# fengpeng-yue/speech-to-speech-translation

Hardware: AMD Instinct MI355X
Metric: mel-frames/sec (fwd+bwd+opt) on Fisher-shaped fbank80->mel80 (higher is better)
Workload: dtype bf16; 1 GPU; s2st_transformer base 12enc/6dec d512 nfps4 + aux ASR/ST(1x64) + CTC, recipe dropouts, max-tokens=20000 Fisher-shaped batches, update-freq 1; parallelism=dp1

## Files before the change

include/s2st_hip.h:

```cpp
#ifndef S2ST_HIP_H
#define S2ST_HIP_H
#include <stdint.h>
#ifdef __cplusplus
extern "C" {
#endif

#define S2ST_OK 0
#define S2ST_ERR_LAUNCH (-1)
#define S2ST_ERR_SHAPE (-2)
#define S2ST_ERR_WORKSPACE (-3)
#define S2ST_ERR_ARG (-4)
#define S2ST_ERR_COMM (-5)

typedef struct { int64_t ld; int64_t bs; int32_t per; int32_t _pad; } s2st_split;

typedef struct {
  const void* p;
  int32_t kmajor;
  int32_t dtype;
  s2st_split sp;
  int64_t zo, zi;
} s2st_gemm_operand;

#define S2ST_F32 0
// ... 90 lines not shown

int s2st_add_pe_f32(const float* x, float* y, const int32_t* pos, const float* table, int32_t rows, int32_t C, float scale, const float* alpha_ptr, float drop_p, uint64_t seed, void* stream);

int s2st_pe_alpha_bwd_f32(const float* dy, const int32_t* pos, const float* table, int32_t rows, int32_t C, float drop_p, uint64_t seed, float* dalpha, void* stream);

int s2st_embed_fwd_f32(const int64_t* tokens, const float* table, float* y, int32_t rows, int32_t C, float scale, void* stream);

int s2st_embed_bwd_f32(const int64_t* tokens, const float* dy, float* dtable, int32_t rows, int32_t C, float scale, int64_t pad, void* stream);
int s2st_embed_bwd_ordered_f32(const int64_t* tokens, const float* dy, float* dtable, int32_t rows, int32_t C, int32_t V, float scale, int64_t pad, void* stream);

int s2st_dropout_f32(const float* x, float* y, int64_t n, float a, float p, uint64_t seed, int32_t accumulate, void* stream);

int s2st_relu_drop_bwd_f32(const float* dy, const float* y, float* dz, int64_t n, float p, void* stream);

int s2st_conv_w_permute_f32(const float* w, float* wf, float* wd, int32_t O, int32_t I, int32_t Kw, void* stream);

int s2st_conv_w_unpermute_acc_f32(const float* dwf, float* dw, int32_t O, int32_t I, int32_t Kw, void* stream);

#define S2ST_BN_TMP_FLOATS(C) (130 * (long)(C))
int s2st_bn_stats_f32(const float* x, int32_t rows, int32_t C, float* mean, float* var, float* run_mean, float* run_var, float momentum, float* tmp, void* stream);

int s2st_bn_apply_f32(const float* x, const float* mean, const float* var, const float* gamma, const float* beta, float* y, s2st_split ysp, const float* resid, int32_t rows, int32_t C, float eps, int32_t tanh_, float drop_p, uint64_t seed, void* stream);

int s2st_bn_bwd_f32(const float* dy, s2st_split dysp, const float* x, const float* mean, const float* var, const float* gamma, const float* beta, float* dx, s2st_split dxsp, float* dgamma, float* dbeta, float* tmp, int32_t rows, int32_t C, float eps, int32_t tanh_, float drop_p, uint64_t seed, void* stream);

int s2st_bn_apply_img_f32(const float* x, const float* mean, const float* var, const float* gamma, const float* beta, float* y, uint16_t* img, int32_t B, int32_t T, int32_t pad, int32_t C, float eps, int32_t tanh_, float drop_p, uint64_t seed, void* stream);

int s2st_bn_stats_apply_f32(const float* x, int32_t rows, int32_t C, float* mean, float* var, float* run_mean, float* run_var, float momentum, float* tmp, const float* gamma, const float* beta, float* y, s2st_split ysp, const float* resid, float eps, int32_t tanh_, float drop_p, uint64_t seed, void* stream);
int s2st_bn_stats_apply_img_f32(const float* x, int32_t B, int32_t T, int32_t pad, int32_t C, float* mean, float* var, float* run_mean, float* run_var, float momentum, float* tmp, const float* gamma, const float* beta, float* y, uint16_t* img, float eps, int32_t tanh_, float drop_p, uint64_t seed, void* stream);

int s2st_bn_bwd_twin_f32(const float* dy, s2st_split dysp, const float* x, const float* mean, const float* var, const float* gamma, const float* beta, float* dx, s2st_split dxsp, float* dgamma, float* dbeta, float* tmp, int32_t rows, int32_t C, float eps, int32_t tanh_, float drop_p, uint64_t seed, uint16_t* dxh, int64_t ldh, void* stream);

// ... 317 lines not shown
```

speech-to-speech-translation_amd/csrc/c_api.cpp:

```cpp
#include <hip/hip_ext.h>
#include "s2st_ops.h"

extern "C" {

int s2st_version(void) { return 100; }

int s2st_experimental_build(void) {
#ifdef S2ST_EXPERIMENTAL
  return 1;
#else
  return 0;
#endif
}

int s2st_device_count(void) {
  int n = 0;
  if (hipGetDeviceCount(&n) != hipSuccess) return 0;
  return n;
}

int s2st_exchange_proxy_f32(const float* bucket, float* scratch, int64_t n, int64_t move_bytes, int32_t wgs, float gbps, void* stream) {
  return s2st_exchange_proxy(bucket, scratch, (long)n, (long)move_bytes, wgs, gbps, (hipStream_t)stream);
}
int s2st_grad_pack_bf16_f32(const float* g, uint16_t* out, int64_t n, void* stream) {
// ... 74 lines not shown
  return s2st_embed_bwd((const long*)tokens, dy, dtable, rows, C, scale, (long)pad, (hipStream_t)stream, V);
}

int s2st_dropout_f32(const float* x, float* y, int64_t n, float a, float p, uint64_t seed, int32_t accumulate, void* stream) {
  return s2st_dropout(x, y, n, a, p, seed, accumulate, (hipStream_t)stream);
}

int s2st_relu_drop_bwd_f32(const float* dy, const float* y, float* dz, int64_t n, float p, void* stream) {
  return s2st_relu_drop_bwd(dy, y, dz, n, p, (hipStream_t)stream);
}

int s2st_conv_w_permute_f32(const float* w, float* wf, float* wd, int32_t O, int32_t I, int32_t Kw, void* stream) {
  return s2st_conv_w_permute(w, wf, wd, O, I, Kw, (hipStream_t)stream);
}

int s2st_conv_w_unpermute_acc_f32(const float* dwf, float* dw, int32_t O, int32_t I, int32_t Kw, void* stream) {
  return s2st_conv_w_unpermute_acc(dwf, dw, O, I, Kw, (hipStream_t)stream);
}

int s2st_bn_stats_f32(const float* x, int32_t rows, int32_t C, float* mean, float* var, float* run_mean, float* run_var, float momentum, float* tmp, void* stream) {
  return s2st_bn_stats(x, rows, C, mean, var, run_mean, run_var, momentum, tmp, (hipStream_t)stream);
}

int s2st_bn_apply_f32(const float* x, const float* mean, const float* var, const float* gamma, const float* beta, float* y, s2st_split ysp, const float* resid, int32_t rows, int32_t C, float eps, int32_t tanh_, float drop_p, uint64_t seed, void* stream) {
  return s2st_bn_apply(x, mean, var, gamma, beta, y, ysp, resid, rows, C, eps, tanh_, drop_p, seed, (hipStream_t)stream);
}

int s2st_bn_bwd_f32(const float* dy, s2st_split dysp, const float* x, const float* mean, const float* var, const float* gamma, const float* beta, float* dx, s2st_split dxsp, float* dgamma, float* dbeta, float* tmp, int32_t rows, int32_t C, float eps, int32_t tanh_, float drop_p, uint64_t seed, void* stream) {
  return s2st_bn_bwd(dy, dysp, x, mean, var, gamma, beta, dx, dxsp, dgamma, dbeta, tmp, rows, C, eps, tanh_, drop_p, seed, (hipStream_t)stream);
}

int s2st_bn_apply_img_f32(const float* x, const float* mean, const float* var, const float* gamma, const float* beta, float* y, uint16_t* img, int32_t B, int32_t T, int32_t pad, int32_t C, float eps, int32_t tanh_, float drop_p, uint64_t seed, void* stream) {
// ... 259 lines not shown
```

speech-to-speech-translation_amd/csrc/elementwise.hip:

```cpp
#include <cstdlib>

#include "s2st_ops.h"
#include "s2st_prof.h"

namespace {

constexpr int EW_BLOCK = 256;

inline unsigned ew_grid(long n, int per_thread = 1) {
  long b = (n + (long)EW_BLOCK * per_thread - 1) / ((long)EW_BLOCK * per_thread);
  return (unsigned)(b < 1 ? 1 : b);
}

__global__ __launch_bounds__(256) void copy_rows_kernel(const float* __restrict__ x, Split xsp,
                                                        float* __restrict__ y, Split ysp, int rows,
                                                        int C4) {
  long i = (long)blockIdx.x * EW_BLOCK + threadIdx.x;
  long n = (long)rows * C4;
  if (i >= n) return;
  int r = (int)(i / C4), c = (int)(i - (long)r * C4);
  reinterpret_cast<float4*>(y + split_off(ysp, r))[c] =
      reinterpret_cast<const float4*>(x + split_off(xsp, r))[c];
}

// ... 408 lines not shown
    else atomicAdd(dbias + cc, v);
  }
}

__global__ __launch_bounds__(256) void axpy_kernel(const float* __restrict__ x,
                                                   float* __restrict__ y, long n, float a) {
  long i = (long)blockIdx.x * EW_BLOCK + threadIdx.x;
  if (i < n) y[i] += a * x[i];
}

__global__ __launch_bounds__(256) void scale_kernel(float* __restrict__ x, long n, float a) {
  long i = (long)blockIdx.x * EW_BLOCK + threadIdx.x;
  if (i < n) x[i] *= a;
}

__global__ __launch_bounds__(256) void conv_w_permute_kernel(const float* __restrict__ w,
                                                             float* __restrict__ wf,
                                                             float* __restrict__ wd, int O, int I,
                                                             int Kw, uint16_t* __restrict__ wfh,
                                                             uint16_t* __restrict__ wdh) {
  long i = (long)blockIdx.x * EW_BLOCK + threadIdx.x;
  long n = (long)O * I * Kw;
  if (i >= n) return;
  int j = (int)(i % Kw);
  int c = (int)((i / Kw) % I);
  int o = (int)(i / ((long)Kw * I));
  float v = w[i];
  const uint16_t vh = (uint16_t)(pack_bf16x4(v, 0.f, 0.f, 0.f).x & 0xffffu);
  if (wf) wf[((long)o * Kw + j) * I + c] = v;
  if (wd) wd[((long)c * Kw + (Kw - 1 - j)) * O + o] = v;
  if (wfh) wfh[((long)o * Kw + j) * I + c] = vh;
  if (wdh) wdh[((long)c * Kw + (Kw - 1 - j)) * O + o] = vh;
}

__global__ __launch_bounds__(256) void conv_w_permute_tiled_kernel(const float* __restrict__ w, float* __restrict__ wf,
                                                                   float* __restrict__ wd, int O, int I, int Kw,
                                                                   uint16_t* __restrict__ wfh, uint16_t* __restrict__ wdh) {
  __shared__ float tile[32][33];
  const int j = blockIdx.z, o0 = blockIdx.y * 32, c0 = blockIdx.x * 32;
  const int tx = threadIdx.x & 31, ty = threadIdx.x >> 5;
#pragma unroll
  for (int r = ty; r < 32; r += 8) {
    const int o = o0 + r, c = c0 + tx;
    float v = 0.f;
    if (o < O && c < I) {
      v = w[((long)o * I + c) * Kw + j];
      const long i = ((long)o * Kw + j) * I + c;
      if (wf) wf[i] = v;
      if (wfh) wfh[i] = (uint16_t)(pack_bf16x4(v, 0.f, 0.f, 0.f).x & 0xffffu);
    }
    tile[r][tx] = v;
  }
  __syncthreads();
  if (!wd && !wdh) return;
#pragma unroll
  for (int r = ty; r < 32; r += 8) {
    const int c = c0 + r, o = o0 + tx;
    if (o < O && c < I) {
      const float v = tile[tx][r];
      const long i = ((long)c * Kw + (Kw - 1 - j)) * O + o;
      if (wd) wd[i] = v;
      if (wdh) wdh[i] = (uint16_t)(pack_bf16x4(v, 0.f, 0.f, 0.f).x & 0xffffu);
    }
  }
}

__global__ __launch_bounds__(256) void conv_w_unpermute_acc_kernel(const float* __restrict__ dwf,
                                                                   float* __restrict__ dw, int O,
                                                                   int I, int Kw, int slabs) {
  long i = (long)blockIdx.x * EW_BLOCK + threadIdx.x;
  long n = (long)O * I * Kw;
  if (i >= n) return;
  int j = (int)(i % Kw);
  int c = (int)((i / Kw) % I);
  int o = (int)(i / ((long)Kw * I));
// ... 636 lines not shown
}

int s2st_axpy(const float* x, float* y, long n, float a, hipStream_t st) {
  if (n <= 0) return 0;
  S2ST_LAUNCH(axpy_kernel, dim3(ew_grid(n)), dim3(EW_BLOCK), 0, st, x, y, n, a);
  return LAUNCH_OK();
}

int s2st_scale(float* x, long n, float a, hipStream_t st) {
  if (n <= 0) return 0;
  S2ST_LAUNCH(scale_kernel, dim3(ew_grid(n)), dim3(EW_BLOCK), 0, st, x, n, a);
  return LAUNCH_OK();
}

int s2st_conv_w_permute(const float* w, float* wf, float* wd, int O, int I, int Kw, hipStream_t st, uint16_t* wfh,
                        uint16_t* wdh) {
  long n = (long)O * I * Kw;
  if (n <= 0) return 0;
  if (O >= 32 && I >= 32 && Kw <= 64) {
    S2ST_LAUNCH(conv_w_permute_tiled_kernel, dim3((I + 31) / 32, (O + 31) / 32, Kw), dim3(256), 0, st, w, wf, wd, O, I, Kw,
                wfh, wdh);
    return LAUNCH_OK();
  }
  S2ST_LAUNCH(conv_w_permute_kernel, dim3(ew_grid(n)), dim3(EW_BLOCK), 0, st, w, wf, wd, O, I, Kw, wfh, wdh);
  return LAUNCH_OK();
}

int s2st_conv_w_unpermute_acc(const float* dwf, float* dw, int O, int I, int Kw, hipStream_t st, int slabs) {
  long n = (long)O * I * Kw;
  if (n <= 0) return 0;
  S2ST_LAUNCH(conv_w_unpermute_acc_kernel, dim3(ew_grid(n)), dim3(EW_BLOCK), 0, st, dwf, dw, O, I, Kw, slabs < 1 ? 1 : slabs);
  return LAUNCH_OK();
}

int s2st_bn_stats(const float* x, int rows, int C, float* mean, float* var, float* run_mean,
                  float* run_var, float momentum, float* tmp, hipStream_t st) {
  if (rows <= 0 || C <= 0) return 0;
  int slabs = 0;
  int rc = colreduce2(ShiftSqF{x, C}, rows, C, nullptr, nullptr, tmp + 2 * (long)C, st, nullptr, nullptr, &slabs);
// ... 93 lines not shown
```

speech-to-speech-translation_amd/csrc/engine.cpp:

```cpp
#include <cmath>
#include <cstdio>
#include <cstdlib>
#include <cstring>
#include <functional>
#include <string>
#include <vector>

#include "s2st_ops.h"
#include <hip/hip_ext.h>

namespace {

struct PInfo {
  std::string name;
  long off, numel;
  int ndim;
  int shape[4];
  int is_buffer;
};

struct Ten {
  float* d = nullptr;
  float* g = nullptr;
  bf16raw* h = nullptr;
// ... 170 lines not shown
  float* dec_selfV(int l) const { return dec_selfK(l) + (long)dec_st.B * dec_st.maxT * c.dec_dim; }
  float* dec_crossKV(int l) const {
    return dec_st.base + (long)c.dec_layers * 2 * dec_st.B * dec_st.maxT * c.dec_dim + (long)l * dec_st.B * dec_st.E * 2 * c.dec_dim;
  }
  bool use_ln_skinny = true;
  bool use_skinny = true;
  bool use_ln_fuse = true;
  bool use_only_h = true;
  bool use_attn_gfuse = true;
  int attn_gfuse_mode = 1;
  bool ordered_sums = true;
  bool use_act_fuse = true;
  bool use_flash = true;
  bool attn_keep_f32 = s2st_env_on("S2ST_ATTN_KEEP_F32");
  bool convnet_fuse = s2st_env_int("S2ST_CONVNET_FUSE", 1) != 0;
  int ffn_act = 1;
  bool is_hubert = false;
  s2st_hubert_config hc{};
  struct HubP {
    long conv_w[8]; long gn_g, gn_b; LNP ln; LinP proj; long pos_w, pos_b; std::vector<EncLayerP> L; LNP enc_ln;
  } hp;
  float* ws_for(hipStream_t s) const { return (side_ && s == side_) ? skws_side : ((chain1_ && s == chain1_) ? skws_c1 : skws); }
  float* skws = nullptr;
  long skws_n = 0;
  bool ph_fresh = false;
  bf16raw* PHT = nullptr;
  bool pht_valid = false;
  struct WT { long off; int N, K; };
  std::vector<WT> wt_list;
  void reg_wt(long off, int N, int K) { if (N % 8 == 0 && K % 8 == 0) wt_list.push_back(WT{off, N, K}); }
// ... 650 lines not shown
```

speech-to-speech-translation_amd/csrc/engine_convnets.h:

```cpp
  ConvW make_conv_scratch(const ConvP& p, bool need_wd, bool tr) {
    ConvW s;
    const bool fm = fast();
    long n = (long)p.O * p.I * p.Kw;
    s.wf = fm ? nullptr : alloc(n);
    s.wd = (need_wd && !fm) ? alloc(n) : nullptr;
    s.dwf = alloc(n, tr);
    bf16raw* wfh = fm ? alloc_h((n + 7) / 8 * 8) : nullptr;
    bf16raw* wdh = fm && need_wd ? alloc_h((n + 7) / 8 * 8) : nullptr;
    if (live() && adam_pending && st_ != side_) adam_wait_upto(p.w + n);
    if (live()) chk(s2st_conv_w_permute(P + p.w, s.wf, s.wd, p.O, p.I, p.Kw, st_, wfh, wdh));
    s.wfh = wfh;
    s.wdh = wdh;
    return s;
  }

  bool bn_bwd_fusable(const Ten* z, int C) const { return fast() && convnet_fuse && C % 4 == 0 && z->hld() % 4 == 0; }
  bf16raw* bn_bwd_image(Ten* z, int B, int T) {
    if (!z->img_want || z->img_stride != 1 || z->img_B != B || z->img_Tout != T || z->img_Th != T + 2 * z->img_pad) return nullptr;
    z->gimg = alloc_h((long)B * z->img_Th * z->cols);
    return z->gimg;
  }

  Ten* postnet(Ten* feat, int B, int D, bool tr, std::vector<ConvW>& csp, float* post_out) {
    const bool fm = fast();
    Ten* cur = feat;
// ... 166 lines not shown
```

speech-to-speech-translation_amd/csrc/engine_ops.h:

```cpp
  Ten* linear(Ten* x, long w, long b, int N, int K, int act = 0, float drop_p = 0.f,
              Ten* resid = nullptr, float* ext_out = nullptr, bool only_h = false, const float* resid_row = nullptr) {
    const int M = x->rows;
    const bool fm = fast();
    const bool skinny = fm && !bt.training && use_skinny && M <= S2ST_SKINNY_MAX_ROWS && K % 32 == 0 && x->d && x->cols == K &&
                        (act == 0 || act == 1 || act == 3);
    only_h = only_h && fast() && use_only_h && N % 8 == 0 && !ext_out && !resid && !skinny;
    Ten* y = newT(M, N, ext_out, !only_h);
    touch(w + (long)N * K);
    if (b >= 0) touch(b + N);
    const uint64_t sd = drop_p > 0.f ? next_seed(S2ST_SITE_LINEAR, drop_p, M, N) : 0;
    if (skinny) {
      const uint64_t* seed_ptr = nullptr;
      if (replay_ && drop_p > 0.f) {
        if (site < 1 || site > 8) { if (!err) err = S2ST_ERR_SHAPE; return y; }
        seed_ptr = replay_->seeds + (site - 1);
      }
      if (live())
        chk(s2st_gemm_skinny(x->d, K, PH + w, K, y->d, N, b >= 0 ? P + b : nullptr, act, drop_p, sd,
                             resid ? resid->d : resid_row, resid ? N : 0, M, N, K, st_, nullptr, nullptr, 1e-5f, seed_ptr,
                             drop_p > 0.f ? dec_row_map : nullptr));
      return y;
    }
    if (replay_ && drop_p > 0.f && !err) err = S2ST_ERR_SHAPE;
    const bf16raw* xh = fm ? half_of(x) : nullptr;
// ... 455 lines not shown
    }
    const int C = xn->cols;
    h.q = linear(xn, l.xa.q_w, l.xa.q_b, C, C, 0, 0.f, nullptr, nullptr, true);
    return h;
  }
  Ten* dec_layer(Ten* x, Ten* encx, const DecLayerP& l, int B, int T, int S, int H, bool pre_ln,
                 const int* self_klen, float* attn_mean_out, Ten* kv_pre = nullptr, const DecHead* head = nullptr) {
    const DecHead h = head ? *head : dec_head(x, l, B, T, H, pre_ln, self_klen);
    x = cross_attn_block(h.q, encx, l.xa, B, T, S, H, bt.enc_lens, h.x, attn_mean_out, kv_pre);
    if (pre_ln) return ffn_block(layernorm(x, l.ln3, nullptr, true), l.fc1, l.fc2, x);
    x = layernorm(x, l.ln2);
    return layernorm(ffn_block(x, l.fc1, l.fc2, x), l.ln3);
  }

  struct ConvIn { float* xh; Ten* src; int Tin; const bf16raw* xhh; };
  struct ConvW { float *wf, *wd, *dwf; const bf16raw *wfh, *wdh; };
  Ten* conv(const ConvIn& in, const ConvP& p, int B, int stride, const ConvW& cw) {
    float *wf = cw.wf, *wd = cw.wd, *dwf = cw.dwf;
    const bf16raw *wfh = cw.wfh, *wdh = cw.wdh;
    const bool fm = fast();
    const int pad = p.Kw / 2;
    const int Tin = in.Tin, Tout = (Tin + 2 * pad - p.Kw) / stride + 1;
    const int Th = Tin + 2 * pad;
    Ten* z = newT(B * Tout, p.O);
    z->img_want = convnet_fuse && fm && p.O % 8 == 0 && in.src && in.src->needs_grad;
    z->img_B = B; z->img_Tout = Tout; z->img_Th = Th; z->img_pad = pad; z->img_stride = stride;
    touch(p.w + (long)p.O * p.I * p.Kw);
    touch(p.b + p.O);
    if (live()) {
      GemmArgs g{};
      g.A = fm ? gemm_rowmajor(in.xhh, (long)stride * p.I) : gemm_rowmajor(in.xh, (long)stride * p.I);
      g.A.sp.per = Tout; g.A.sp.bs = (long)Th * p.I;
      g.B = fm ? gemm_rowmajor(wfh, (long)p.Kw * p.I) : gemm_rowmajor(wf, (long)p.Kw * p.I);
      g.C = gemm_out(z->d, p.O);
      g.ep = gemm_epi_default();
      g.ep.bias = P + p.b;
      g.M = B * Tout; g.N = p.O; g.K = p.Kw * p.I; g.batch = 1; g.zdiv = 1; g.precise = c.precise;
      chk(s2st_gemm(g, st_));
    }
    ConvP pp = p;
    ConvIn in2 = in;
    tape.push_back([=]() {
      if (!z->g) return;
      const int M = B * Tout;
      const bf16raw* dzh = fm ? ghalf_of(z) : nullptr;
      float* cpart = ordered_sums ? alloc(s2st_colsum_scratch_floats(M, pp.O)) : nullptr;
      const bool no_dgrad = !(in2.src && in2.src->needs_grad);
      const bool direct = fm && pp.O % 8 == 0;
      const bool need_img = !no_dgrad;
      float* up = (need_img && !direct) ? alloc((long)B * Th * pp.O, true) : nullptr;
      const bool have_img = need_img && direct && z->gimg;
      bf16raw* upd = have_img ? z->gimg : ((need_img && direct) ? alloc_h((long)B * Th * pp.O) : nullptr);
      if (need_img && !have_img && live()) {
        Split xs{(long)pp.O, 0, 0, 0};
        Split ys{(long)stride * pp.O, (long)Th * pp.O, Tout, 0};
        if (direct) {
          chk(s2st_halo_image_bf16(dzh, z->hld(), upd, B, Tout, Th, pp.O, pad, stride, st_));
        } else {
          chk(s2st_copy_rows(z->g, xs, up + (long)pad * pp.O, ys, M, pp.O, st_));
        }
      }
      if (live()) {
        hipStream_t side_st = fm ? fork_side() : st_;
        hipStream_t ws_st = (fm && !no_dgrad) ? side_st : st_;
        {
          GemmArgs g{};
          g.A = fm ? gemm_colmajor(dzh, z->hld()) : gemm_colmajor(z->g, pp.O);
          g.B = fm ? gemm_colmajor(in2.xhh, (long)stride * pp.I) : gemm_colmajor(in2.xh, (long)stride * pp.I);
          g.B.sp.per = Tout; g.B.sp.bs = (long)Th * pp.I;
          g.C = gemm_out(dwf, (long)pp.Kw * pp.I);
          g.ep = gemm_epi_default();
          g.ep.accumulate = 1;
          g.ws = ws_for(ws_st); g.ws_floats = skws_n;
          g.M = pp.O; g.N = pp.Kw * pp.I; g.K = M; g.batch = 1; g.zdiv = 1; g.precise = c.precise;
          chk(s2st_gemm(g, ws_st));
        }
        {
          int slabs = 0;
          chk(s2st_colsum(z->g, pp.O, M, pp.O, G + pp.b, 1, side_st, cpart, cpart ? &slabs : nullptr));
          if (cpart) add_fold(cpart, slabs, pp.O, G + pp.b);
        }
        chk(s2st_conv_w_unpermute_acc(dwf, G + pp.w, pp.O, pp.I, pp.Kw, ws_st, 1));
      }
      if (!no_dgrad) {
        bool acc;
        float* dx = gradbuf(in2.src, acc);
        const bf16raw* uph = direct ? upd : (fm ? cast_buf(up, (long)B * Th * pp.O) : nullptr);
        if (live()) {
          GemmArgs g{};
          g.A = fm ? gemm_rowmajor(uph, pp.O) : gemm_rowmajor(up, pp.O);
          g.A.sp.per = Tin; g.A.sp.bs = (long)Th * pp.O;
          g.B = fm ? gemm_rowmajor(wdh, (long)pp.Kw * pp.O) : gemm_rowmajor(wd, (long)pp.Kw * pp.O);
          g.C = gemm_out(dx, pp.I);
          g.ep = gemm_epi_default();
          g.ep.accumulate = acc ? 1 : 0;
          g.ws = ws_for(st_); g.ws_floats = skws_n;
          g.M = B * Tin; g.N = pp.I; g.K = pp.Kw * pp.O; g.batch = 1; g.zdiv = 1; g.precise = c.precise;
          chk(s2st_gemm(g, st_));
        }
      }
    });
    return z;
  }
// ... 82 lines not shown
```

speech-to-speech-translation_amd/csrc/engine_step.h:

```cpp
  bool use_streamk = s2st_env_on("S2ST_GEMM_STREAMK");
  void reset_call() {
    pending_wgrad.clear();
    pending_lnfold = s2st_lnfold_table{};
    s2st_gemm_streamk_unbind_all();
    for (Ten* t : tens) delete t;
    tens.clear();
    tape.clear();
    tape_aware.clear();
    forked_ = false;
    in_region_ = false;
    marks.clear();
    ws_top = 0;
    ws_peak = 0;
    oom = false;
    err = 0;
    site = 0;
    site_log.clear();
    xattn0_idx = 0;
    tail_bwd_on_side = tail_side_ = dec_early_active = false;
    site_ctx[0] = 0;
    param_watermark = 0;
    next_segment = 0;
    skws = nullptr; skws_n = 0; skws_side = nullptr;
  }
// ... 53 lines not shown
    skws_side = fm && side_allowed ? alloc(skws_n) : skws;
    skws_c1 = fm && chain1_ && nchains == 2 ? alloc(skws_n) : skws;
    if (fm && tr && use_streamk) {
      float* sk0 = alloc(S2ST_STREAMK_SCRATCH_FLOATS);
      float* sk1 = side_allowed ? alloc(S2ST_STREAMK_SCRATCH_FLOATS) : nullptr;
      if (live()) {
        hipMemsetAsync(sk0, 0, 4096, st_);
        s2st_gemm_streamk_bind(st_, sk0, S2ST_STREAMK_SCRATCH_FLOATS);
        if (sk1 && side_) {
          hipMemsetAsync(sk1, 0, 4096, st_);
          s2st_gemm_streamk_bind(side_, sk1, S2ST_STREAMK_SCRATCH_FLOATS);
        }
      }
    }
    typedef ConvW ConvScratch;
    auto conv_scratch = [&](const ConvP& p, bool need_wd) { return make_conv_scratch(p, need_wd, tr); };
    ConvScratch cs0{}, cs1{};
    std::vector<ConvScratch> cst;
    if (c.text_input) {
      for (auto& pc : enc_conv) cst.push_back(conv_scratch(pc, true));
    } else {
      cs0 = conv_scratch(sub[0], false);
      cs1 = conv_scratch(sub[1], true);
    }
    std::vector<ConvScratch> csp;
    {
      const bool post_on_side = fm && side_ && ev_taps_ && ev_kv_ && live() && hoist_kv && !stop_after_encoder &&
                                c.dec_layers > 0;
      hipStream_t main_st = st_;
      if (post_on_side) st_ = fork_side();
      for (auto& pc : post_conv) csp.push_back(conv_scratch(pc, true));
      st_ = main_st;
    }

    const bool kv_side_ok = side_ && side_events_ && hoist_kv && !stop_after_encoder;
    const bool dec_early = tr && fm && (dec_overlap & 1) && kv_side_ok && !two_chains && !c.text_input && !c.s2t_mode &&
                           c.dec_layers > 0 && bt.prev && !(dec_spk >= 0 && bt.speaker);
    struct {
// ... 419 lines not shown
```

speech-to-speech-translation_amd/csrc/gemm.hip:

```cpp
#include <cstdio>
#include <cstdlib>
#include <cstring>
#include <vector>

#include "s2st_ops.h"
#include "s2st_prof.h"

namespace {

constexpr int BK = 32;
constexpr int LDS_ROW = 80;

__device__ __forceinline__ constexpr int kslot(int k) {
  return (k & 19) | ((k & 4) << 1) | ((k & 8) >> 1);
}

template <bool KM, int ROWS, bool VEC>
struct TileLoader {
  static constexpr int NLD = ROWS * 8 / 256;
  static constexpr int RQ = ROWS / 4;
  static constexpr int PITCH = KM ? LDS_ROW : (2 * ROWS + 32);
  static constexpr int BYTES = KM ? ROWS * LDS_ROW : BK * (2 * ROWS + 32);
  float r[NLD][4];
  long off[NLD];
// ... 265 lines not shown
    Agg* f = nullptr;
    for (auto& a : aggs) if (strcmp(a.tag, r.tag) == 0) { f = &a; break; }
    if (!f) { aggs.push_back(Agg{r.tag, 0, 0, 0, 0}); f = &aggs.back(); }
    f->n += 1; f->us += e * 1e3; f->work += r.work; f->work2 += r.work2;
  }
  g_prof.clear();
  long o = 0;
  for (auto& a : aggs) {
    int w = snprintf(out + o, cap > o ? (size_t)(cap - o) : 0, "%s\t%ld\t%.3f\t%.6e\t%.6e\n", a.tag, a.n, a.us, a.work, a.work2);
    if (w < 0 || o + w >= cap) return -1;
    o += w;
  }
  return o;
}

int s2st_gemm(GemmArgs g, hipStream_t st, int* tile_out) {
  if (tile_out) *tile_out = 0;
  if (g.M <= 0 || g.N <= 0 || g.batch <= 0) return 0;
  if (g.A.dtype != g.B.dtype) return S2ST_ERR_ARG;
  const bool bf16_in = g.A.dtype == S2ST_BF16;
  if (bf16_in && g.precise) return S2ST_ERR_ARG;
  if (!bf16_in && (g.C.h || !g.C.p)) return S2ST_ERR_ARG;
  if (g.zdiv <= 0) g.zdiv = 1;
  if (bf16_in) {
    int tile = 0;
    const int rc = s2st_gemm_bf16(g, st, &tile);
    if (tile_out) *tile_out = tile;
    return rc;
  }
  g.avec = vec_ok(g.A, g.M, g.K) ? 1 : 0;
  g.bvec = vec_ok(g.B, g.N, g.K) ? 1 : 0;
  const bool vec = g.avec && g.bvec;
  auto tiles = [&](int bm, int bn) {
    return (long)((g.M + bm - 1) / bm) * ((g.N + bn - 1) / bn) * g.batch;
  };
  bool linear_epi = !g.ep.act && g.ep.drop_p == 0.f;
  bool wgrad_like = g.ep.accumulate && linear_epi && g.K >= 16 * BK;
  bool big = vec && !g.precise && (tiles(128, 128) >= 192 || (wgrad_like && g.M >= 128 && g.N >= 128));
  int bm = big ? 128 : 64, bn = bm;
  long nt = tiles(bm, bn);
  g.splitk = 1;
// ... 24 lines not shown
```

speech-to-speech-translation_amd/csrc/gemm_bf16.hip:

```cpp
#include "gemm_bf16_tile.h"
#include "gemm_bf16_launch.h"

namespace {

template <int BM, int BN, bool AKM, bool BKM, bool VEC>
__global__ __launch_bounds__(256) void gemm_bf16_kernel(GemmArgs g) {
  constexpr int WM = BM / 2, WN = BN / 2, TM = WM / 16, TN = WN / 16;
  typedef Stage<AKM, BM, VEC> LA;
  typedef Stage<BKM, BN, VEC> LB;
  constexpr int A_BYTES = LA::BYTES, B_BYTES = LB::BYTES, STAGE = A_BYTES + B_BYTES;
  __shared__ __attribute__((aligned(16))) unsigned char smem[2 * STAGE];

  const int tid = threadIdx.x;
  const int wave = tid >> 6, lane = tid & 63;
  const int wm = wave >> 1, wn = wave & 1;

  const int nwg = gridDim.x;
  int id = blockIdx.x;
  {
    const int x = id & 7, q = nwg >> 3, r = nwg & 7;
    id = (x < r ? x * (q + 1) : r * (q + 1) + (x - r) * q) + (id >> 3);
  }
  const int tile_m = id / g.tiles_n, tile_n = id - tile_m * g.tiles_n;
  const int m0 = tile_m * BM, n0 = tile_n * BN;
// ... 672 lines not shown
      for (int j = 0; j < 8; ++j) v[j] = *reinterpret_cast<const float4*>(sp + (long)min(sb + j, splitk - 1) * sstride);
#pragma unroll
      for (int j = 0; j < 8; ++j)
        if (sb + j < splitk) { a.x += v[j].x; a.y += v[j].y; a.z += v[j].z; a.w += v[j].w; }
    }
    *reinterpret_cast<float4*>(cp) = a;
  } else {
    for (int r = 0; r < 4 && n + r < N; ++r) {
      float a = accumulate ? cp[r] : 0.f;
      for (int s = 0; s < splitk; ++s) a += sp[s * sstride + r];
      cp[r] = a;
    }
  }
}

template <int BM, int BN, bool VEC>
int launch_staged(const GemmArgs& g, dim3 grid, hipStream_t st) {
  return with_layouts(g, [&](auto a, auto b) {
    constexpr bool AKM = decltype(a)::value, BKM = decltype(b)::value;
    return launch_configured<GEMM_STAGED, BM, BN, AKM, BKM, VEC>(gemm_bf16_kernel<BM, BN, AKM, BKM, VEC>, 0, grid, 256, st, g);
  });
}

constexpr bool kExperimental =
#ifdef S2ST_EXPERIMENTAL
    true;
#else
    false;
#endif
static_assert(GEMM_BK == BK, "the plan prices the kernels' K-step");
// ... 99 lines not shown
    grp.n = 1;
    grp.g[0] = g;
#ifdef S2ST_EXPERIMENTAL
    rc |= launch_persistent<128, 128>(grp, false, 1, st);
    rc |= launch_persistent<128, 64>(grp, false, 1, st);
    rc |= launch_persistent<256, 128>(grp, false, 1, st);
    rc |= launch_ring<256, 128>(g, grid, st);
#endif
    rc |= launch_group_ring(grp, st);
  }
  rc |= s2st_gemm_bf16_w4_preload(st);
  rc |= s2st_gemm_bf16_p4_preload(st);
  return rc || hipGetLastError() != hipSuccess ? -1 : 0;
}

int s2st_gemm_bf16(GemmArgs g, hipStream_t st, int* tile_out) {
  const GemmSwitches sw = gemm_switches(SW_SINGLE);
  const GemmPlan p = plan_single(g, sw, gemm_chip(sw), sk_scratch(st) != nullptr);
  if (p.error) return p.error;
  g.avec = g.bvec = p.vec;
  g.cvec = p.cvec;
  g.splitk = p.splitk;
  g.kchunk = p.kchunk;
  g.tiles_n = p.tiles_n;
  g.slab = p.use_slab ? g.ws : nullptr;
  if (tile_out) *tile_out = p.bm * 1000 + p.bn;
  const dim3 grid(p.grid_x, p.grid_y, 1);
  const bool wide = p.bn == 128;
  int rc = S2ST_ERR_ARG;
  switch (p.form) {
    case GEMM_STAGED:
      rc = !p.vec ? launch_staged<64, 64, false>(g, grid, st) : p.bm == 64 ? launch_staged<64, 64, true>(g, grid, st)
           : wide ? launch_staged<128, 128, true>(g, grid, st) : launch_staged<128, 64, true>(g, grid, st);
      break;
// ... 1 lines not shown
      rc = p.bm == 160 ? launch_ring<160, 64>(g, grid, st) : p.bm == 64 ? launch_ring<64, 64>(g, grid, st)
           : wide ? launch_ring<128, 128>(g, grid, st) : launch_ring<128, 64>(g, grid, st);
      break;
    case GEMM_W4: rc = s2st_gemm_bf16_w4(g, p.bm, p.bn, grid, st); break;
    case GEMM_P4: rc = s2st_gemm_bf16_p4(g, grid, st); break;
#ifdef S2ST_EXPERIMENTAL
    case GEMM_RING_256x128: rc = launch_ring<256, 128>(g, grid, st); break;
    case GEMM_PERSISTENT:
      rc = wide ? launch_persistent<128, 128>(group_of(&g, p), p.sk, p.grid_x, st)
                : launch_persistent<128, 64>(group_of(&g, p), p.sk, p.grid_x, st);
      break;
#endif
    default: break;
  }
  if (rc) return rc;
  if (p.use_slab) {
    const long nthr = (long)g.M * ((g.N + 3) / 4);
    const double by = 4.0 * g.M * g.N * g.batch * (g.splitk + 1 + (g.ep.accumulate ? 1 : 0));
    s2st_launch("splitk_reduce_kernel", by, 0.0, splitk_reduce_kernel, dim3((unsigned)((nthr + 255) / 256), g.batch),
                dim3(256), 0, st, (const float*)g.slab, g.C, g.M, g.N, g.splitk, g.zdiv, g.ep.accumulate);
  }
  return hipGetLastError() == hipSuccess ? 0 : -1;
}

int s2st_gemm_bf16_plan(const GemmArgs* list, int n, int ncu, int slots160, bool sk_bound, s2st_gemm_plan_info* out) {
  const GemmSwitches sw = gemm_switches(n ? SW_GROUP : SW_SINGLE);
  const GemmChip chip = gemm_chip(sw, ncu, slots160);
  GemmPlan p;
  if (list[0].A.dtype != S2ST_BF16 || list[0].B.dtype != S2ST_BF16 || list[0].precise) p.error = S2ST_ERR_ARG;
  else if (n == 0) p = plan_single(list[0], sw, chip, sk_bound);
  else {
    for (int i = 0; i < n && !p.error; ++i)
      if (!group_member_ok(list[i], sw)) p.error = S2ST_ERR_SHAPE;
    if (!p.error) p = plan_group(list, n, sw, chip, sk_bound);
  }
  *out = s2st_gemm_plan_info{p.error};
  if (p.error) return 0;
// ... 220 lines not shown
```

speech-to-speech-translation_amd/csrc/s2st_ops.h:

```cpp
#pragma once
#include <cstdlib>
static inline const char* s2st_env_str(const char* name) { return getenv(name); }
static inline int s2st_env_int(const char* name, int dflt) { const char* e = getenv(name); return e ? atoi(e) : dflt; }
static inline bool s2st_env_on(const char* name) { return s2st_env_int(name, 0) != 0; }

#include <hip/hip_runtime.h>
#include <stdint.h>
#include "s2st_common.h"
#include "gemm_bf16_plan.h"

typedef s2st_gemm_out GemmOut;
typedef s2st_gemm_epilogue GemmEpilogue;

inline GemmOperand gemm_rowmajor(const float* p, long ld) {
  GemmOperand o;
  o.p = p; o.kmajor = 1; o.dtype = S2ST_F32; o.sp.ld = ld; o.sp.bs = 0; o.sp.per = 0; o.sp._pad = 0;
  o.zo = o.zi = 0;
  return o;
}
inline GemmOperand gemm_colmajor(const float* p, long ld) {
  GemmOperand o = gemm_rowmajor(p, ld);
  o.kmajor = 0;
  return o;
}
// ... 23 lines not shown

struct GemmGroup {
  int n, total;
  int tile0[S2ST_GROUP_MAX + 1];
  GemmArgs g[S2ST_GROUP_MAX];
  int sk, epoch;
  int xcd_global;
  int* sk_ctr;
  int* sk_flag;
  float* sk_part;
};
void s2st_gemm_streamk_bind(hipStream_t st, float* scratch, long floats);
void s2st_gemm_streamk_unbind_all();
bool s2st_gemm_group_ok(const GemmArgs& g);
int s2st_gemm_bf16_group(const GemmArgs* list, int n, hipStream_t st);
int s2st_gemm(GemmArgs g, hipStream_t st, int* tile_out = nullptr );
int s2st_gemm_bf16(GemmArgs g, hipStream_t st, int* tile_out);
int s2st_gemm_bf16_plan(const GemmArgs* list, int n, int ncu, int slots160, bool sk_bound, s2st_gemm_plan_info* out);
int s2st_gemm_skinny(const float* A, long lda, const bf16raw* W, long ldw, float* C, long ldc, const float* bias, int act,
                     float drop_p, uint64_t seed, const float* resid, long ldr, int M, int N, int K, hipStream_t st,
                     const float* ln_g = nullptr, const float* ln_b = nullptr, float ln_eps = 1e-5f ,
                     const uint64_t* seed_ptr = nullptr ,
                     const int* row_map = nullptr );
#define S2ST_SKINNY_MAX_ROWS 256
int s2st_gemm_bf16_w4(const GemmArgs& g, int bm, int bn, dim3 grid, hipStream_t st);
int s2st_gemm_bf16_w4_slots160();
int s2st_gemm_bf16_w4_group(const GemmGroup& grp, hipStream_t st);
int s2st_gemm_bf16_w4_preload(hipStream_t st);
int s2st_gemm_bf16_p4(const GemmArgs& g, dim3 grid, hipStream_t st);
int s2st_gemm_bf16_p4_preload(hipStream_t st);
int s2st_gemm_bf16_preload(hipStream_t st);
void s2st_profile_enable_impl(int on);
// ... 77 lines not shown
                   hipStream_t st);
int s2st_embed_bwd(const long* tokens, const float* dy, float* dtable, int rows, int C, float scale,
                   long pad, hipStream_t st, int V = 0 );
int s2st_dropout(const float* x, float* y, long n, float a, float p, uint64_t seed, int accumulate,
                 hipStream_t st);
int s2st_relu_drop_bwd(const float* dy, const float* y, float* dz, long n, float p,
                       hipStream_t st);
int s2st_linear_bwd_prep(const float* dy, const float* y, const uint16_t* yb , int mode,
                         float p, uint64_t seed, uint16_t* dph, long ldp, float* dpre, float* dbias, int M, int N,
                         hipStream_t st, float* part = nullptr ,
                         int* slabs_out = nullptr );
long s2st_linear_bwd_prep_scratch_floats(int M, int N, long ldp);
int s2st_axpy(const float* x, float* y, long n, float a, hipStream_t st);
int s2st_scale(float* x, long n, float a, hipStream_t st);
int s2st_conv_w_permute(const float* w, float* wf, float* wd, int O, int I, int Kw, hipStream_t st,
                        uint16_t* wfh = nullptr, uint16_t* wdh = nullptr );
int s2st_conv_w_unpermute_acc(const float* dwf, float* dw, int O, int I, int Kw, hipStream_t st, int slabs = 1);
int s2st_bn_stats(const float* x, int rows, int C, float* mean, float* var, float* run_mean,
                  float* run_var, float momentum, float* tmp, hipStream_t st);
int s2st_bn_apply(const float* x, const float* mean, const float* var, const float* gamma,
                  const float* beta, float* y, Split ysp, const float* resid, int rows, int C,
                  float eps, int tanh_, float drop_p, uint64_t seed, hipStream_t st);
int s2st_bn_apply_img(const float* x, const float* mean, const float* var, const float* gamma, const float* beta, float* y,
                      uint16_t* img, int B, int T, int pad, int C, float eps, int tanh_, float drop_p, uint64_t seed,
                      hipStream_t st);
int s2st_bn_stats_apply(const float* x, int rows, int C, float* mean, float* var, float* run_mean, float* run_var,
                        float momentum, float* tmp, const float* gamma, const float* beta, float* y, Split ysp,
                        const float* resid, float eps, int tanh_, float drop_p, uint64_t seed, hipStream_t st);
int s2st_bn_stats_apply_img(const float* x, int B, int T, int pad, int C, float* mean, float* var, float* run_mean,
                            float* run_var, float momentum, float* tmp, const float* gamma, const float* beta, float* y,
                            uint16_t* img, float eps, int tanh_, float drop_p, uint64_t seed, hipStream_t st);
// ... 151 lines not shown
```

Measured before the change: 1.505 million mel-frames/s.

## Split stride-2 conv dgrad into phase GEMMs and fuse wgrad split-K unpermute

For the stride-2, kernel-5 subsampling conv, the input-gradient GEMM is split into two phase GEMMs with 3 and 2 taps over a dense, unstrided halo image. This avoids multiplying by the zeros that the strided upsampled image would insert, and the weight permute reorders taps into phase slots to match. The weight-gradient GEMM can also fold its split-K reduction straight into the unpermuted dw layout, which skips the separate dwf buffer and the unpermute kernel. The cost is added layout complexity, plus a memset or accumulate-mode change when no slab is used.

Result: no change. 1.519 million mel-frames/s (median of 6 runs) (+0.9%).

```diff
diff --git a/include/s2st_hip.h b/include/s2st_hip.h
--- a/include/s2st_hip.h
+++ b/include/s2st_hip.h
@@ -128,8 +128,12 @@
 int s2st_relu_drop_bwd_f32(const float* dy, const float* y, float* dz, int64_t n, float p, void* stream);
 
 int s2st_conv_w_permute_f32(const float* w, float* wf, float* wd, int32_t O, int32_t I, int32_t Kw, void* stream);
+int s2st_conv_w_permute_phases_f32(const float* w, float* wd, uint16_t* wdh, int32_t O, int32_t I, int32_t Kw, void* stream);
 
 int s2st_conv_w_unpermute_acc_f32(const float* dwf, float* dw, int32_t O, int32_t I, int32_t Kw, void* stream);
+
+int s2st_splitk_reduce_f32(const float* slab, float* c, int64_t ldc, int32_t M, int32_t N, int32_t splitk, int32_t accumulate, void* stream);
+int s2st_splitk_reduce_conv_w_f32(const float* slab, float* dw, int32_t splitk, int32_t O, int32_t I, int32_t Kw, void* stream);
 
 #define S2ST_BN_TMP_FLOATS(C) (130 * (long)(C))
 int s2st_bn_stats_f32(const float* x, int32_t rows, int32_t C, float* mean, float* var, float* run_mean, float* run_var, float momentum, float* tmp, void* stream);
diff --git a/speech-to-speech-translation_amd/csrc/c_api.cpp b/speech-to-speech-translation_amd/csrc/c_api.cpp
--- a/speech-to-speech-translation_amd/csrc/c_api.cpp
+++ b/speech-to-speech-translation_amd/csrc/c_api.cpp
@@ -112,8 +112,20 @@
   return s2st_conv_w_permute(w, wf, wd, O, I, Kw, (hipStream_t)stream);
 }
 
+int s2st_conv_w_permute_phases_f32(const float* w, float* wd, uint16_t* wdh, int32_t O, int32_t I, int32_t Kw, void* stream) {
+  return s2st_conv_w_permute(w, nullptr, wd, O, I, Kw, (hipStream_t)stream, nullptr, wdh, 1);
+}
+
 int s2st_conv_w_unpermute_acc_f32(const float* dwf, float* dw, int32_t O, int32_t I, int32_t Kw, void* stream) {
   return s2st_conv_w_unpermute_acc(dwf, dw, O, I, Kw, (hipStream_t)stream);
+}
+
+int s2st_splitk_reduce_f32(const float* slab, float* c, int64_t ldc, int32_t M, int32_t N, int32_t splitk, int32_t accumulate, void* stream) {
+  return s2st_splitk_reduce(slab, c, (long)ldc, M, N, splitk, accumulate, (hipStream_t)stream);
+}
+
+int s2st_splitk_reduce_conv_w_f32(const float* slab, float* dw, int32_t splitk, int32_t O, int32_t I, int32_t Kw, void* stream) {
+  return s2st_splitk_reduce_conv_w(slab, dw, splitk, O, I, Kw, (hipStream_t)stream);
 }
 
 int s2st_bn_stats_f32(const float* x, int32_t rows, int32_t C, float* mean, float* var, float* run_mean, float* run_var, float momentum, float* tmp, void* stream) {
diff --git a/speech-to-speech-translation_amd/csrc/elementwise.hip b/speech-to-speech-translation_amd/csrc/elementwise.hip
--- a/speech-to-speech-translation_amd/csrc/elementwise.hip
+++ b/speech-to-speech-translation_amd/csrc/elementwise.hip
@@ -446,11 +446,15 @@
   if (i < n) x[i] *= a;
 }
 
+__device__ __forceinline__ int conv_wd_tap_slot(int jf, int Kw, int phases) {
+  return phases ? ((jf & 1) ? (Kw + 1) / 2 + (jf >> 1) : (jf >> 1)) : jf;
+}
+
 __global__ __launch_bounds__(256) void conv_w_permute_kernel(const float* __restrict__ w,
                                                              float* __restrict__ wf,
                                                              float* __restrict__ wd, int O, int I,
                                                              int Kw, uint16_t* __restrict__ wfh,
-                                                             uint16_t* __restrict__ wdh) {
+                                                             uint16_t* __restrict__ wdh, int phases) {
   long i = (long)blockIdx.x * EW_BLOCK + threadIdx.x;
   long n = (long)O * I * Kw;
   if (i >= n) return;
@@ -460,14 +464,16 @@
   float v = w[i];
   const uint16_t vh = (uint16_t)(pack_bf16x4(v, 0.f, 0.f, 0.f).x & 0xffffu);
   if (wf) wf[((long)o * Kw + j) * I + c] = v;
-  if (wd) wd[((long)c * Kw + (Kw - 1 - j)) * O + o] = v;
+  const long di = ((long)c * Kw + conv_wd_tap_slot(Kw - 1 - j, Kw, phases)) * O + o;
+  if (wd) wd[di] = v;
   if (wfh) wfh[((long)o * Kw + j) * I + c] = vh;
-  if (wdh) wdh[((long)c * Kw + (Kw - 1 - j)) * O + o] = vh;
+  if (wdh) wdh[di] = vh;
 }
 
 __global__ __launch_bounds__(256) void conv_w_permute_tiled_kernel(const float* __restrict__ w, float* __restrict__ wf,
                                                                    float* __restrict__ wd, int O, int I, int Kw,
-                                                                   uint16_t* __restrict__ wfh, uint16_t* __restrict__ wdh) {
+                                                                   uint16_t* __restrict__ wfh, uint16_t* __restrict__ wdh,
+                                                                   int phases) {
   __shared__ float tile[32][33];
   const int j = blockIdx.z, o0 = blockIdx.y * 32, c0 = blockIdx.x * 32;
   const int tx = threadIdx.x & 31, ty = threadIdx.x >> 5;
@@ -490,7 +496,7 @@
     const int c = c0 + r, o = o0 + tx;
     if (o < O && c < I) {
       const float v = tile[tx][r];
-      const long i = ((long)c * Kw + (Kw - 1 - j)) * O + o;
+      const long i = ((long)c * Kw + conv_wd_tap_slot(Kw - 1 - j, Kw, phases)) * O + o;
       if (wd) wd[i] = v;
       if (wdh) wdh[i] = (uint16_t)(pack_bf16x4(v, 0.f, 0.f, 0.f).x & 0xffffu);
     }
@@ -1157,15 +1163,15 @@
 }
 
 int s2st_conv_w_permute(const float* w, float* wf, float* wd, int O, int I, int Kw, hipStream_t st, uint16_t* wfh,
-                        uint16_t* wdh) {
+                        uint16_t* wdh, int phases) {
   long n = (long)O * I * Kw;
   if (n <= 0) return 0;
   if (O >= 32 && I >= 32 && Kw <= 64) {
     S2ST_LAUNCH(conv_w_permute_tiled_kernel, dim3((I + 31) / 32, (O + 31) / 32, Kw), dim3(256), 0, st, w, wf, wd, O, I, Kw,
-                wfh, wdh);
+                wfh, wdh, phases);
     return LAUNCH_OK();
   }
-  S2ST_LAUNCH(conv_w_permute_kernel, dim3(ew_grid(n)), dim3(EW_BLOCK), 0, st, w, wf, wd, O, I, Kw, wfh, wdh);
+  S2ST_LAUNCH(conv_w_permute_kernel, dim3(ew_grid(n)), dim3(EW_BLOCK), 0, st, w, wf, wd, O, I, Kw, wfh, wdh, phases);
   return LAUNCH_OK();
 }
 
diff --git a/speech-to-speech-translation_amd/csrc/engine.cpp b/speech-to-speech-translation_amd/csrc/engine.cpp
--- a/speech-to-speech-translation_amd/csrc/engine.cpp
+++ b/speech-to-speech-translation_amd/csrc/engine.cpp
@@ -208,6 +208,8 @@
   bool use_flash = true;
   bool attn_keep_f32 = s2st_env_on("S2ST_ATTN_KEEP_F32");
   bool convnet_fuse = s2st_env_int("S2ST_CONVNET_FUSE", 1) != 0;
+  bool conv_wgrad_direct = s2st_env_int("S2ST_CONV_WGRAD_DIRECT", 1) != 0;
+  bool conv_dgrad_phases = s2st_env_int("S2ST_CONV_DGRAD_PHASES", 1) != 0;
   int ffn_act = 1;
   bool is_hubert = false;
   s2st_hubert_config hc{};
diff --git a/speech-to-speech-translation_amd/csrc/engine_convnets.h b/speech-to-speech-translation_amd/csrc/engine_convnets.h
--- a/speech-to-speech-translation_amd/csrc/engine_convnets.h
+++ b/speech-to-speech-translation_amd/csrc/engine_convnets.h
@@ -1,14 +1,18 @@
-  ConvW make_conv_scratch(const ConvP& p, bool need_wd, bool tr) {
+  bool conv_dgrad_by_phase(const ConvP& p, int stride) const {
+    return fast() && conv_dgrad_phases && stride == 2 && p.Kw == 5 && p.O % GEMM_BK == 0;
+  }
+  ConvW make_conv_scratch(const ConvP& p, bool need_wd, bool tr, int stride = 1) {
     ConvW s;
     const bool fm = fast();
+    s.dphase = need_wd && conv_dgrad_by_phase(p, stride) ? 1 : 0;
     long n = (long)p.O * p.I * p.Kw;
     s.wf = fm ? nullptr : alloc(n);
     s.wd = (need_wd && !fm) ? alloc(n) : nullptr;
-    s.dwf = alloc(n, tr);
+    s.dwf = alloc(n, tr && !(fm && conv_wgrad_direct));
     bf16raw* wfh = fm ? alloc_h((n + 7) / 8 * 8) : nullptr;
     bf16raw* wdh = fm && need_wd ? alloc_h((n + 7) / 8 * 8) : nullptr;
     if (live() && adam_pending && st_ != side_) adam_wait_upto(p.w + n);
-    if (live()) chk(s2st_conv_w_permute(P + p.w, s.wf, s.wd, p.O, p.I, p.Kw, st_, wfh, wdh));
+    if (live()) chk(s2st_conv_w_permute(P + p.w, s.wf, s.wd, p.O, p.I, p.Kw, st_, wfh, wdh, s.dphase));
     s.wfh = wfh;
     s.wdh = wdh;
     return s;
diff --git a/speech-to-speech-translation_amd/csrc/engine_ops.h b/speech-to-speech-translation_amd/csrc/engine_ops.h
--- a/speech-to-speech-translation_amd/csrc/engine_ops.h
+++ b/speech-to-speech-translation_amd/csrc/engine_ops.h
@@ -493,7 +493,7 @@
   }
 
   struct ConvIn { float* xh; Ten* src; int Tin; const bf16raw* xhh; };
-  struct ConvW { float *wf, *wd, *dwf; const bf16raw *wfh, *wdh; };
+  struct ConvW { float *wf, *wd, *dwf; const bf16raw *wfh, *wdh; int dphase;  };
   Ten* conv(const ConvIn& in, const ConvP& p, int B, int stride, const ConvW& cw) {
     float *wf = cw.wf, *wd = cw.wd, *dwf = cw.dwf;
     const bf16raw *wfh = cw.wfh, *wdh = cw.wdh;
@@ -503,7 +503,9 @@
     const int Th = Tin + 2 * pad;
     Ten* z = newT(B * Tout, p.O);
     z->img_want = convnet_fuse && fm && p.O % 8 == 0 && in.src && in.src->needs_grad;
-    z->img_B = B; z->img_Tout = Tout; z->img_Th = Th; z->img_pad = pad; z->img_stride = stride;
+    const bool phases = cw.dphase && fm && stride == 2 && p.Kw == 5;
+    const int iTh = phases ? Tout + 2 : Th, ipad = phases ? 1 : pad, istride = phases ? 1 : stride;
+    z->img_B = B; z->img_Tout = Tout; z->img_Th = iTh; z->img_pad = ipad; z->img_stride = istride;
     touch(p.w + (long)p.O * p.I * p.Kw);
     touch(p.b + p.O);
     if (live()) {
@@ -529,12 +531,12 @@
       const bool need_img = !no_dgrad;
       float* up = (need_img && !direct) ? alloc((long)B * Th * pp.O, true) : nullptr;
       const bool have_img = need_img && direct && z->gimg;
-      bf16raw* upd = have_img ? z->gimg : ((need_img && direct) ? alloc_h((long)B * Th * pp.O) : nullptr);
+      bf16raw* upd = have_img ? z->gimg : ((need_img && direct) ? alloc_h((long)B * iTh * pp.O) : nullptr);
       if (need_img && !have_img && live()) {
         Split xs{(long)pp.O, 0, 0, 0};
         Split ys{(long)stride * pp.O, (long)Th * pp.O, Tout, 0};
         if (direct) {
-          chk(s2st_halo_image_bf16(dzh, z->hld(), upd, B, Tout, Th, pp.O, pad, stride, st_));
+          chk(s2st_halo_image_bf16(dzh, z->hld(), upd, B, Tout, iTh, pp.O, ipad, istride, st_));
         } else {
           chk(s2st_copy_rows(z->g, xs, up + (long)pad * pp.O, ys, M, pp.O, st_));
         }
@@ -542,6 +544,7 @@
       if (live()) {
         hipStream_t side_st = fm ? fork_side() : st_;
         hipStream_t ws_st = (fm && !no_dgrad) ? side_st : st_;
+        GemmConvWCombine cwc{G + pp.w, pp.O, pp.I, pp.Kw, 0};
         {
           GemmArgs g{};
           g.A = fm ? gemm_colmajor(dzh, z->hld()) : gemm_colmajor(z->g, pp.O);
@@ -552,20 +555,34 @@
           g.ep.accumulate = 1;
           g.ws = ws_for(ws_st); g.ws_floats = skws_n;
           g.M = pp.O; g.N = pp.Kw * pp.I; g.K = M; g.batch = 1; g.zdiv = 1; g.precise = c.precise;
-          chk(s2st_gemm(g, ws_st));
+          chk(s2st_gemm(g, ws_st, nullptr, (fm && conv_wgrad_direct) ? &cwc : nullptr));
         }
         {
           int slabs = 0;
           chk(s2st_colsum(z->g, pp.O, M, pp.O, G + pp.b, 1, side_st, cpart, cpart ? &slabs : nullptr));
           if (cpart) add_fold(cpart, slabs, pp.O, G + pp.b);
         }
-        chk(s2st_conv_w_unpermute_acc(dwf, G + pp.w, pp.O, pp.I, pp.Kw, ws_st, 1));
+        if (!cwc.used) chk(s2st_conv_w_unpermute_acc(dwf, G + pp.w, pp.O, pp.I, pp.Kw, ws_st, 1));
       }
       if (!no_dgrad) {
         bool acc;
         float* dx = gradbuf(in2.src, acc);
         const bf16raw* uph = direct ? upd : (fm ? cast_buf(up, (long)B * Th * pp.O) : nullptr);
-        if (live()) {
+        for (int ph = 0; ph < 2 && phases && live(); ++ph) {
+          const int Mp = ph ? Tin / 2 : (Tin + 1) / 2, taps = ph ? 2 : 3;
+          GemmArgs g{};
+          g.A = gemm_rowmajor(uph + (long)ph * pp.O, pp.O);
+          g.A.sp.per = Mp; g.A.sp.bs = (long)iTh * pp.O;
+          g.B = gemm_rowmajor(wdh + (long)ph * 3 * pp.O, (long)pp.Kw * pp.O);
+          g.C = gemm_out(dx + (long)ph * pp.I, 2L * pp.I);
+          g.C.sp.per = Mp; g.C.sp.bs = (long)Tin * pp.I;
+          g.ep = gemm_epi_default();
+          g.ep.accumulate = acc ? 1 : 0;
+          g.ws = ws_for(st_); g.ws_floats = skws_n;
+          g.M = B * Mp; g.N = pp.I; g.K = taps * pp.O; g.batch = 1; g.zdiv = 1; g.precise = c.precise;
+          chk(s2st_gemm(g, st_));
+        }
+        if (live() && !phases) {
           GemmArgs g{};
           g.A = fm ? gemm_rowmajor(uph, pp.O) : gemm_rowmajor(up, pp.O);
           g.A.sp.per = Tin; g.A.sp.bs = (long)Th * pp.O;
diff --git a/speech-to-speech-translation_amd/csrc/engine_step.h b/speech-to-speech-translation_amd/csrc/engine_step.h
--- a/speech-to-speech-translation_amd/csrc/engine_step.h
+++ b/speech-to-speech-translation_amd/csrc/engine_step.h
@@ -91,14 +91,14 @@
       }
     }
     typedef ConvW ConvScratch;
-    auto conv_scratch = [&](const ConvP& p, bool need_wd) { return make_conv_scratch(p, need_wd, tr); };
+    auto conv_scratch = [&](const ConvP& p, bool need_wd, int stride = 1) { return make_conv_scratch(p, need_wd, tr, stride); };
     ConvScratch cs0{}, cs1{};
     std::vector<ConvScratch> cst;
     if (c.text_input) {
       for (auto& pc : enc_conv) cst.push_back(conv_scratch(pc, true));
     } else {
       cs0 = conv_scratch(sub[0], false);
-      cs1 = conv_scratch(sub[1], true);
+      cs1 = conv_scratch(sub[1], true, 2);
     }
     std::vector<ConvScratch> csp;
     {
diff --git a/speech-to-speech-translation_amd/csrc/gemm.hip b/speech-to-speech-translation_amd/csrc/gemm.hip
--- a/speech-to-speech-translation_amd/csrc/gemm.hip
+++ b/speech-to-speech-translation_amd/csrc/gemm.hip
@@ -303,8 +303,9 @@
   return o;
 }
 
-int s2st_gemm(GemmArgs g, hipStream_t st, int* tile_out) {
+int s2st_gemm(GemmArgs g, hipStream_t st, int* tile_out, GemmConvWCombine* cw) {
   if (tile_out) *tile_out = 0;
+  if (cw && g.A.dtype != S2ST_BF16) return S2ST_ERR_ARG;
   if (g.M <= 0 || g.N <= 0 || g.batch <= 0) return 0;
   if (g.A.dtype != g.B.dtype) return S2ST_ERR_ARG;
   const bool bf16_in = g.A.dtype == S2ST_BF16;
@@ -313,7 +314,7 @@
   if (g.zdiv <= 0) g.zdiv = 1;
   if (bf16_in) {
     int tile = 0;
-    const int rc = s2st_gemm_bf16(g, st, &tile);
+    const int rc = s2st_gemm_bf16(g, st, &tile, cw);
     if (tile_out) *tile_out = tile;
     return rc;
   }
diff --git a/speech-to-speech-translation_amd/csrc/gemm_bf16.hip b/speech-to-speech-translation_amd/csrc/gemm_bf16.hip
--- a/speech-to-speech-translation_amd/csrc/gemm_bf16.hip
+++ b/speech-to-speech-translation_amd/csrc/gemm_bf16.hip
@@ -710,6 +710,28 @@
   }
 }
 
+__global__ __launch_bounds__(256) void splitk_reduce_conv_w_kernel(const float* __restrict__ slab, float* __restrict__ dw,
+                                                                   int splitk, int O, int I, int Kw) {
+  const long i = (long)blockIdx.x * 256 + threadIdx.x;
+  if (i >= (long)O * I) return;
+  const int o = (int)(i / I), c = (int)(i - (long)o * I);
+  const long sstride = (long)O * Kw * I;
+  const float* sp = slab + (long)o * Kw * I + c;
+  float* dp = dw + i * Kw;
+  for (int j = 0; j < Kw; ++j, sp += I) {
+    float a = 0.f;
+    for (int sb = 0; sb < splitk; sb += 8) {
+      float v[8];
+#pragma unroll
+      for (int k = 0; k < 8; ++k) v[k] = sp[(long)min(sb + k, splitk - 1) * sstride];
+#pragma unroll
+      for (int k = 0; k < 8; ++k)
+        if (sb + k < splitk) a += v[k];
+    }
+    dp[j] += a;
+  }
+}
+
 template <int BM, int BN, bool VEC>
 int launch_staged(const GemmArgs& g, dim3 grid, hipStream_t st) {
   return with_layouts(g, [&](auto a, auto b) {
@@ -839,10 +861,17 @@
   return rc || hipGetLastError() != hipSuccess ? -1 : 0;
 }
 
-int s2st_gemm_bf16(GemmArgs g, hipStream_t st, int* tile_out) {
+int s2st_gemm_bf16(GemmArgs g, hipStream_t st, int* tile_out, GemmConvWCombine* cw) {
   const GemmSwitches sw = gemm_switches(SW_SINGLE);
   const GemmPlan p = plan_single(g, sw, gemm_chip(sw), sk_scratch(st) != nullptr);
   if (p.error) return p.error;
+  if (cw) {
+    if (!g.ep.accumulate || g.batch != 1 || g.M != cw->O || g.N != cw->Kw * cw->I || g.C.sp.ld != g.N || g.C.sp.per > 0)
+      return S2ST_ERR_ARG;
+    cw->used = p.use_slab ? 1 : 0;
+    if (p.splitk == 1) g.ep.accumulate = 0;
+    else if (!p.use_slab && hipMemsetAsync(g.C.p, 0, sizeof(float) * g.M * g.N, st) != hipSuccess) return S2ST_ERR_LAUNCH;
+  }
   g.avec = g.bvec = p.vec;
   g.cvec = p.cvec;
   g.splitk = p.splitk;
@@ -874,13 +903,35 @@
     default: break;
   }
   if (rc) return rc;
-  if (p.use_slab) {
+  if (p.use_slab && cw) {
+    const long nthr = (long)cw->O * cw->I;
+    const double by = 4.0 * g.M * g.N * (g.splitk + 2);
+    s2st_launch("splitk_reduce_conv_w_kernel", by, 0.0, splitk_reduce_conv_w_kernel, dim3((unsigned)((nthr + 255) / 256)),
+                dim3(256), 0, st, (const float*)g.slab, cw->dw, g.splitk, cw->O, cw->I, cw->Kw);
+  } else if (p.use_slab) {
     const long nthr = (long)g.M * ((g.N + 3) / 4);
     const double by = 4.0 * g.M * g.N * g.batch * (g.splitk + 1 + (g.ep.accumulate ? 1 : 0));
     s2st_launch("splitk_reduce_kernel", by, 0.0, splitk_reduce_kernel, dim3((unsigned)((nthr + 255) / 256), g.batch),
                 dim3(256), 0, st, (const float*)g.slab, g.C, g.M, g.N, g.splitk, g.zdiv, g.ep.accumulate);
   }
   return hipGetLastError() == hipSuccess ? 0 : -1;
+}
+
+int s2st_splitk_reduce(const float* slab, float* c, long ldc, int M, int N, int splitk, int accumulate, hipStream_t st) {
+  if (M <= 0 || N <= 0) return 0;
+  if (splitk < 1) return S2ST_ERR_ARG;
+  const long nthr = (long)M * ((N + 3) / 4);
+  s2st_launch("splitk_reduce_kernel", 4.0 * M * N * (splitk + 1 + (accumulate ? 1 : 0)), 0.0, splitk_reduce_kernel,
+              dim3((unsigned)((nthr + 255) / 256), 1), dim3(256), 0, st, slab, gemm_out(c, ldc), M, N, splitk, 1, accumulate);
+  return hipGetLastError() == hipSuccess ? 0 : S2ST_ERR_LAUNCH;
+}
+int s2st_splitk_reduce_conv_w(const float* slab, float* dw, int splitk, int O, int I, int Kw, hipStream_t st) {
+  if (O <= 0 || I <= 0 || Kw <= 0) return 0;
+  if (splitk < 1) return S2ST_ERR_ARG;
+  const long nthr = (long)O * I;
+  s2st_launch("splitk_reduce_conv_w_kernel", 4.0 * O * I * Kw * (splitk + 2), 0.0, splitk_reduce_conv_w_kernel,
+              dim3((unsigned)((nthr + 255) / 256)), dim3(256), 0, st, slab, dw, splitk, O, I, Kw);
+  return hipGetLastError() == hipSuccess ? 0 : S2ST_ERR_LAUNCH;
 }
 
 int s2st_gemm_bf16_plan(const GemmArgs* list, int n, int ncu, int slots160, bool sk_bound, s2st_gemm_plan_info* out) {
diff --git a/speech-to-speech-translation_amd/csrc/s2st_ops.h b/speech-to-speech-translation_amd/csrc/s2st_ops.h
--- a/speech-to-speech-translation_amd/csrc/s2st_ops.h
+++ b/speech-to-speech-translation_amd/csrc/s2st_ops.h
@@ -61,8 +61,12 @@
 void s2st_gemm_streamk_unbind_all();
 bool s2st_gemm_group_ok(const GemmArgs& g);
 int s2st_gemm_bf16_group(const GemmArgs* list, int n, hipStream_t st);
-int s2st_gemm(GemmArgs g, hipStream_t st, int* tile_out = nullptr );
-int s2st_gemm_bf16(GemmArgs g, hipStream_t st, int* tile_out);
+struct GemmConvWCombine { float* dw; int O, I, Kw; int used; };
+int s2st_gemm(GemmArgs g, hipStream_t st, int* tile_out = nullptr ,
+              GemmConvWCombine* cw = nullptr);
+int s2st_gemm_bf16(GemmArgs g, hipStream_t st, int* tile_out, GemmConvWCombine* cw = nullptr);
+int s2st_splitk_reduce(const float* slab, float* c, long ldc, int M, int N, int splitk, int accumulate, hipStream_t st);
+int s2st_splitk_reduce_conv_w(const float* slab, float* dw, int splitk, int O, int I, int Kw, hipStream_t st);
 int s2st_gemm_bf16_plan(const GemmArgs* list, int n, int ncu, int slots160, bool sk_bound, s2st_gemm_plan_info* out);
 int s2st_gemm_skinny(const float* A, long lda, const bf16raw* W, long ldw, float* C, long ldc, const float* bias, int act,
                      float drop_p, uint64_t seed, const float* resid, long ldr, int M, int N, int K, hipStream_t st,
@@ -170,7 +174,7 @@
 int s2st_axpy(const float* x, float* y, long n, float a, hipStream_t st);
 int s2st_scale(float* x, long n, float a, hipStream_t st);
 int s2st_conv_w_permute(const float* w, float* wf, float* wd, int O, int I, int Kw, hipStream_t st,
-                        uint16_t* wfh = nullptr, uint16_t* wdh = nullptr );
+                        uint16_t* wfh = nullptr, uint16_t* wdh = nullptr , int phases = 0);
 int s2st_conv_w_unpermute_acc(const float* dwf, float* dw, int O, int I, int Kw, hipStream_t st, int slabs = 1);
 int s2st_bn_stats(const float* x, int rows, int C, float* mean, float* var, float* run_mean,
                   float* run_var, float momentum, float* tmp, hipStream_t st);
```
